# jaymarichua/Applestar

Hardware: AMD Instinct MI355X
Metric: learner samples/sec (AlphaStar policy) (higher is better)
Workload: dtype fp32

## Files before the change

applestar_amd/csrc/bindings.cpp:

```cpp
#include <cstring>
#include <cstdlib>
#include <map>
#include <string>
#include <torch/extension.h>
#include <c10/hip/HIPStream.h>
#include <c10/hip/HIPGuard.h>

#include "kernels.h"

namespace {

hipStream_t stream() { return c10::hip::getCurrentHIPStream().stream(); }

int dt(const at::Tensor& t) {
  if (t.scalar_type() == at::kFloat) return as::DT_F32;
  if (t.scalar_type() == at::kBFloat16) return as::DT_BF16;
  TORCH_CHECK(false, "applestar_amd: unsupported dtype ", t.scalar_type());
}

void check_cuda(const at::Tensor& t, const char* name) {
  TORCH_CHECK(t.is_cuda(), "applestar_amd: ", name, " must be a GPU tensor");
  TORCH_CHECK(t.is_contiguous(), "applestar_amd: ", name, " must be contiguous");
}

// ... 1365 lines not shown
                        static_cast<int>(K), static_cast<int>(act), stream());
  else
    as::gemm_bf16(a.data_ptr(), b.data_ptr(), bp, rp, out.data_ptr(), M, static_cast<int>(N), static_cast<int>(K),
                  static_cast<int>(act), stream());
  return out;
}

at::Tensor gemm_bf16_small(const at::Tensor& a, const at::Tensor& b, const c10::optional<at::Tensor>& bias,
                           const c10::optional<at::Tensor>& res, int64_t act) {
  return gemm_bf16_impl(a, b, bias, res, act, true);
}
at::Tensor gemm_bf16(const at::Tensor& a, const at::Tensor& b, const c10::optional<at::Tensor>& bias,
                     const c10::optional<at::Tensor>& res, int64_t act) {
  return gemm_bf16_impl(a, b, bias, res, act, false);
}

at::Tensor small_gemm(const at::Tensor& a, const at::Tensor& b, const c10::optional<at::Tensor>& bias,
                      const c10::optional<at::Tensor>& res, const c10::optional<at::Tensor>& amask, int64_t mask_mode,
                      int64_t act) {
  check_cuda(a, "a");
  check_cuda(b, "b");
  const bool bf = a.scalar_type() == at::kBFloat16;
  TORCH_CHECK((bf || a.scalar_type() == at::kFloat) && b.scalar_type() == a.scalar_type() && a.dim() == 2 &&
                  b.dim() == 2 && a.is_contiguous() && b.is_contiguous() && a.size(1) == b.size(1),
              "small_gemm: contiguous A [M,K], B [N,K] of one dtype (fp32 / bf16)");
  const int64_t M = a.size(0), K = a.size(1), N = b.size(0);
  TORCH_CHECK(M * K < (1LL << 31) && N * K < (1LL << 31) && M * N < (1LL << 31), "small_gemm: too large");
  TORCH_CHECK(mask_mode >= 0 && mask_mode <= 2 && (act == 0 || act == 1 || act == 2 || act == 4), "small_gemm: codes");
  const float* bp = nullptr;
  if (bias && bias->defined()) {
    TORCH_CHECK(bias->scalar_type() == at::kFloat && bias->numel() == N && bias->is_contiguous() && bias->is_cuda(),
                "small_gemm: fp32 bias [N]");
    bp = bias->data_ptr<float>();
  }
  const void* rp = nullptr;
  if (res && res->defined()) {
    TORCH_CHECK(res->scalar_type() == a.scalar_type() && res->numel() == M * N && res->is_contiguous() && res->is_cuda(),
                "small_gemm: res [M, N] in A's dtype");
    rp = res->data_ptr();
  }
  TORCH_CHECK(act != 4 || rp != nullptr, "small_gemm: the DRELU epilogue masks by res");
  const void* mp = nullptr;
  if (amask && amask->defined() && mask_mode > 0) {
    TORCH_CHECK(amask->scalar_type() == a.scalar_type() && amask->numel() == M * K && amask->is_contiguous() &&
                    amask->is_cuda(), "small_gemm: amask [M, K] in A's dtype");
    mp = amask->data_ptr();
  }
  c10::hip::HIPGuard g(a.device().index());
  auto out = at::empty({M, N}, a.options());
  as::small_nt(a.data_ptr(), b.data_ptr(), bp, rp, mp, static_cast<int>(mask_mode), out.data_ptr(), M,
               static_cast<int>(N), static_cast<int>(K), static_cast<int>(act), bf, stream());
  return out;
}

at::Tensor small_gemm_splitk(const at::Tensor& a, const at::Tensor& b, const c10::optional<at::Tensor>& bias,
                             int64_t act) {
  check_cuda(a, "a");
  check_cuda(b, "b");
  const bool bf = a.scalar_type() == at::kBFloat16;
  TORCH_CHECK((bf || a.scalar_type() == at::kFloat) && b.scalar_type() == a.scalar_type() && a.dim() == 2 &&
                  b.dim() == 2 && a.is_contiguous() && b.is_contiguous() && a.size(1) == b.size(1),
              "small_gemm_splitk: contiguous A [M,K], B [N,K] of one dtype (fp32 / bf16)");
  const int64_t M = a.size(0), K = a.size(1), N = b.size(0);
  TORCH_CHECK(M * K < (1LL << 31) && N * K < (1LL << 31) && M * N < (1LL << 28), "small_gemm_splitk: too large");
  TORCH_CHECK(act == 0 || act == 1 || act == 2, "small_gemm_splitk: act code");
  const float* bp = nullptr;
  if (bias && bias->defined()) {
    TORCH_CHECK(bias->scalar_type() == at::kFloat && bias->numel() == N && bias->is_contiguous() && bias->is_cuda(),
                "small_gemm_splitk: fp32 bias [N]");
    bp = bias->data_ptr<float>();
  }
  c10::hip::HIPGuard g(a.device().index());
  auto out = at::empty({M, N}, a.options());
  const int S = as::small_nt_splits(M, static_cast<int>(N), static_cast<int>(K));
  if (S <= 1) {
    as::small_nt(a.data_ptr(), b.data_ptr(), bp, nullptr, nullptr, 0, out.data_ptr(), M, static_cast<int>(N),
                 static_cast<int>(K), static_cast<int>(act), bf, stream());
    return out;
  }
  auto part = at::empty({S, M, N}, a.options().dtype(at::kFloat));
  as::small_nt_splitk(a.data_ptr(), b.data_ptr(), bp, part.data_ptr<float>(), S, out.data_ptr(), M,
                      static_cast<int>(N), static_cast<int>(K), static_cast<int>(act), bf, stream());
  return out;
}

std::vector<at::Tensor> small_wgrad(const at::Tensor& dy, const at::Tensor& x, const c10::optional<at::Tensor>& ymask,
                                    int64_t mask_mode, bool want_bias, bool out_bf16) {
  check_cuda(dy, "dy");
  check_cuda(x, "x");
  const bool bf = dy.scalar_type() == at::kBFloat16;
  TORCH_CHECK((bf || dy.scalar_type() == at::kFloat) && x.scalar_type() == dy.scalar_type() && dy.dim() == 2 &&
                  x.dim() == 2 && dy.is_contiguous() && x.is_contiguous() && dy.size(0) == x.size(0),
              "small_wgrad: contiguous dy [R, N], x [R, K] of one dtype");
  TORCH_CHECK(!out_bf16 || bf, "small_wgrad: bf16 output needs bf16 inputs");
  TORCH_CHECK(mask_mode >= 0 && mask_mode <= 2, "small_wgrad: mask code");
  const int64_t R = dy.size(0), N = dy.size(1), K = x.size(1);
  TORCH_CHECK(R * N < (1LL << 31) && R * K < (1LL << 31) && N * K < (1LL << 31), "small_wgrad: too large");
  const void* mp = nullptr;
  if (ymask && ymask->defined() && mask_mode > 0) {
    TORCH_CHECK(ymask->scalar_type() == dy.scalar_type() && ymask->numel() == R * N && ymask->is_contiguous() &&
                    ymask->is_cuda(), "small_wgrad: ymask [R, N] in dy's dtype");
    mp = ymask->data_ptr();
  }
  c10::hip::HIPGuard g(dy.device().index());
  auto opts = out_bf16 ? dy.options() : dy.options().dtype(at::kFloat);
  auto dw = at::empty({N, K}, opts);
  at::Tensor db = want_bias ? at::empty({N}, opts) : at::Tensor();
  if (R == 0) {
    dw.zero_();
    if (want_bias) db.zero_();
    return {dw, db};
  }
  as::small_tn(dy.data_ptr(), x.data_ptr(), mp, static_cast<int>(mask_mode), dw.data_ptr(),
               want_bias ? db.data_ptr() : nullptr, R, static_cast<int>(N), static_cast<int>(K), bf, out_bf16, stream());
  return {dw, db};
}

std::vector<at::Tensor> wgrad_f32(const at::Tensor& dy, const at::Tensor& x, int64_t cin, bool want_bias,
                                  const c10::optional<at::Tensor>& out) {
  check_cuda(dy, "dy");
  check_cuda(x, "x");
  TORCH_CHECK(dy.scalar_type() == at::kFloat && x.scalar_type() == at::kFloat, "wgrad_f32: fp32 dy / x");
  TORCH_CHECK(dy.dim() == 2 && dy.is_contiguous() && x.is_contiguous(), "wgrad_f32: contiguous dy [R, N], x");
  const int64_t R = dy.size(0), N = dy.size(1);
  int64_t K, H = 1, W = 1;
  if (cin > 0) {
    TORCH_CHECK(x.dim() == 4 && x.size(3) == cin && x.size(0) * x.size(1) * x.size(2) == R, "wgrad_f32: x NHWC");
    H = x.size(1);
    W = x.size(2);
    K = 9 * cin;
    TORCH_CHECK(cin % 4 == 0, "wgrad_f32: Cin % 4");
  } else {
    TORCH_CHECK(x.dim() == 2 && x.size(0) == R, "wgrad_f32: x [R, K]");
    K = x.size(1);
  }
  TORCH_CHECK(N % 4 == 0 && K % 4 == 0, "wgrad_f32: N and K must be multiples of 4");
  TORCH_CHECK(R * N * 4 < 0x7ffffff0LL && x.numel() * 4 < 0x7ffffff0LL, "wgrad_f32: tensor too large");
  c10::hip::HIPGuard g(dy.device().index());
  auto opts = dy.options();
  const int64_t NK = N * K, stride = NK + (want_bias ? N : 0);
  at::Tensor flat;
  if (out && out->defined()) {
    TORCH_CHECK(out->scalar_type() == at::kFloat && out->is_contiguous() && out->numel() == stride &&
                out->device() == dy.device(), "wgrad_f32: out must be a contiguous fp32 [N K (+ N)] buffer");
    flat = *out;
  }
  if (R == 0) {
    if (flat.defined()) {
      flat.zero_();
      return {flat.narrow(0, 0, NK).view({N, K}), want_bias ? flat.narrow(0, NK, N) : at::Tensor()};
    }
    return {at::zeros({N, K}, opts), want_bias ? at::zeros({N}, opts) : at::Tensor()};
  }
  const int S = as::wgrad_f32_splits(R, static_cast<int>(N), static_cast<int>(K));
  auto part = (S == 1 && flat.defined()) ? flat.view({1, stride}) : at::empty({S, stride}, opts);
  as::wgrad_f32(dy.data_ptr<float>(), x.data_ptr<float>(), part.data_ptr<float>(),
                want_bias ? part.data_ptr<float>() + NK : nullptr, stride, R, static_cast<int>(N), static_cast<int>(K),
                static_cast<int>(H), static_cast<int>(W), static_cast<int>(cin), S, stream());
  if (S == 1) {
    if (!flat.defined()) flat = part.view({stride});
  } else {
    if (!flat.defined()) flat = at::empty({stride}, opts);
    as::column_reduce(part.data_ptr<float>(), flat.data_ptr<float>(), S, static_cast<int>(stride), stream());
  }
  return {flat.narrow(0, 0, NK).view({N, K}), want_bias ? flat.narrow(0, NK, N) : at::Tensor()};
}

std::vector<at::Tensor> wgrad(const at::Tensor& dy, const at::Tensor& x, int64_t cin, bool want_bias, bool bf16_out) {
  check_cuda(dy, "dy");
  check_cuda(x, "x");
  TORCH_CHECK(dy.scalar_type() == at::kBFloat16 && x.scalar_type() == at::kBFloat16, "wgrad: bf16 dy / x");
  TORCH_CHECK(dy.dim() == 2, "wgrad: dy [R, N]");
  TORCH_CHECK(dy.is_contiguous() && x.is_contiguous(), "wgrad: dy and x must be contiguous");
  const int64_t R = dy.size(0), N = dy.size(1);
  int64_t K, H = 1, W = 1;
  if (cin > 0) {
    TORCH_CHECK(x.dim() == 4 && x.size(3) == cin && x.size(0) * x.size(1) * x.size(2) == R, "wgrad: x NHWC");
    H = x.size(1);
    W = x.size(2);
    K = 9 * cin;
    TORCH_CHECK(cin % 8 == 0, "wgrad: Cin % 8");
  } else {
    TORCH_CHECK(x.dim() == 2 && x.size(0) == R, "wgrad: x [R, K]");
    K = x.size(1);
  }
  TORCH_CHECK(N % 8 == 0 && K % 8 == 0, "wgrad: N and K must be multiples of 8");
  TORCH_CHECK(R * N * 2 < 0x7ffffff0LL && x.numel() * 2 < 0x7ffffff0LL, "wgrad: tensor too large");
  c10::hip::HIPGuard g(dy.device().index());
  const int S = R > 0 ? as::wgrad_splits(R, static_cast<int>(N), static_cast<int>(K)) : 1;
  auto opts = dy.options().dtype(at::kFloat);
  if (R == 0) {
    auto zo = bf16_out ? dy.options() : opts;
    return {at::zeros({N, K}, zo), want_bias ? at::zeros({N}, zo) : at::Tensor()};
  }
  const int64_t NK = N * K, stride = NK + (want_bias ? N : 0);
  if (bf16_out && S == 1) {
    auto flat = at::empty({stride}, dy.options());
    as::wgrad(dy.data_ptr(), x.data_ptr(), reinterpret_cast<float*>(flat.data_ptr()),
              want_bias ? reinterpret_cast<float*>(static_cast<at::BFloat16*>(flat.data_ptr()) + NK) : nullptr, 0, R,
              static_cast<int>(N), static_cast<int>(K), static_cast<int>(H), static_cast<int>(W), static_cast<int>(cin),
              1, stream(), true);
    return {flat.narrow(0, 0, NK).view({N, K}), want_bias ? flat.narrow(0, NK, N) : at::Tensor()};
  }
  auto part = at::empty({S, stride}, opts);
  static const bool nan_fill = [] {
    const char* e = std::getenv("APPLESTAR_WGRAD_NANFILL");
    return e != nullptr && e[0] == '1';
  }();
  if (nan_fill) part.fill_(std::numeric_limits<float>::quiet_NaN());
  as::wgrad(dy.data_ptr(), x.data_ptr(), part.data_ptr<float>(), want_bias ? part.data_ptr<float>() + NK : nullptr,
            stride, R, static_cast<int>(N), static_cast<int>(K), static_cast<int>(H), static_cast<int>(W),
            static_cast<int>(cin), S, stream());
  at::Tensor flat;
  if (bf16_out && S <= 1024) {
    flat = at::empty({stride}, dy.options());
    as::column_reduce_bf16(part.data_ptr<float>(), flat.data_ptr(), S, static_cast<int>(stride), stream());
  } else if (S == 1) {
    flat = part.view({stride});
  } else {
    flat = at::empty({stride}, opts);
    as::column_reduce(part.data_ptr<float>(), flat.data_ptr<float>(), S, static_cast<int>(stride), stream());
  }
  if (bf16_out && flat.scalar_type() != at::kBFloat16) flat = flat.to(at::kBFloat16);
  return {flat.narrow(0, 0, NK).view({N, K}), want_bias ? flat.narrow(0, NK, N) : at::Tensor()};
}

namespace {
int idx_code(const at::Tensor& t) {
  if (t.scalar_type() == at::kShort) return 0;
  if (t.scalar_type() == at::kInt) return 1;
  TORCH_CHECK(t.scalar_type() == at::kLong, "bo_encoder: index dtype int16 / int32 / int64");
  return 2;
}

as::BoWeights bo_weights(const std::vector<at::Tensor>& p, int* wdt) {
  TORCH_CHECK(p.size() == 2 + 12 * as::kBoLayers, "bo_encoder: 38 parameter tensors");
  const auto lin_t = p[0].scalar_type();
  TORCH_CHECK(lin_t == at::kFloat || lin_t == at::kBFloat16, "bo_encoder: linear dtype");
  auto lin = [&](const at::Tensor& t, int64_t numel) {
    TORCH_CHECK(t.is_cuda() && t.is_contiguous() && t.scalar_type() == lin_t && t.numel() == numel,
                "bo_encoder: linear parameter (dtype / shape / contiguity)");
    return static_cast<const void*>(t.data_ptr());
  };
  auto ln = [&](const at::Tensor& t) {
    TORCH_CHECK(t.is_cuda() && t.is_contiguous() && t.scalar_type() == at::kFloat && t.numel() == 64,
                "bo_encoder: LayerNorm parameter fp32 [64]");
    return t.data_ptr<float>();
  };
  as::BoWeights w;
  w.w0 = lin(p[0], 64 * 214);
  w.b0 = lin(p[1], 64);
  for (int l = 0; l < as::kBoLayers; ++l) {
    const int o = 2 + 12 * l;
    w.ln1w[l] = ln(p[o]);
    w.ln1b[l] = ln(p[o + 1]);
    w.wqkv[l] = lin(p[o + 2], 48 * 64);
    w.bqkv[l] = lin(p[o + 3], 48);
    w.wp[l] = lin(p[o + 4], 64 * 16);
    w.bp[l] = lin(p[o + 5], 64);
    w.ln2w[l] = ln(p[o + 6]);
    w.ln2b[l] = ln(p[o + 7]);
    w.w1[l] = lin(p[o + 8], 128 * 64);
    w.b1[l] = lin(p[o + 9], 128);
    w.w2[l] = lin(p[o + 10], 64 * 128);
    w.b2[l] = lin(p[o + 11], 64);
  }
  *wdt = lin_t == at::kBFloat16 ? as::DT_BF16 : as::DT_F32;
  return w;
}
}

std::vector<at::Tensor> bo_encoder_fwd(const at::Tensor& bo, const at::Tensor& loc, const std::vector<at::Tensor>& params,
                                       bool save) {
  check_cuda(bo, "bo");
  check_cuda(loc, "loc");
  TORCH_CHECK(bo.dim() == 2 && bo.size(1) == as::kBoTokens && bo.is_contiguous() && loc.sizes() == bo.sizes() &&
                  loc.is_contiguous() && loc.scalar_type() == bo.scalar_type(),
              "bo_encoder: bo / loc [B, 20] contiguous, same dtype");
  int wdt = 0;
  const as::BoWeights w = bo_weights(params, &wdt);
  const int64_t B = bo.size(0);
  c10::hip::HIPGuard g(bo.device().index());
  auto opts = bo.options().dtype(at::kFloat);
  auto out = at::empty({B, 64}, opts);
  at::Tensor rec;
  if (save) rec = at::empty({B, as::kBoLayers, as::kBoRecord}, opts);
  as::bo_encoder_fwd(bo.data_ptr(), loc.data_ptr(), idx_code(bo), w, wdt, out.data_ptr<float>(),
                     save ? rec.data_ptr<float>() : nullptr, B, stream());
  return {out, rec};
}

at::Tensor bo_encoder_bwd(const at::Tensor& bo, const at::Tensor& loc, const std::vector<at::Tensor>& params,
                          const at::Tensor& save, const at::Tensor& dmean, bool ordered) {
  check_cuda(dmean, "dmean");
  const int64_t B = bo.size(0);
  TORCH_CHECK(dmean.scalar_type() == at::kFloat && dmean.is_contiguous() && dmean.numel() == B * 64,
              "bo_encoder_bwd: dmean fp32 [B, 64]");
  TORCH_CHECK(save.scalar_type() == at::kFloat && save.numel() == B * as::kBoLayers * as::kBoRecord,
              "bo_encoder_bwd: saved record");
  int wdt = 0;
  const as::BoWeights w = bo_weights(params, &wdt);
  c10::hip::HIPGuard g(bo.device().index());
  const int reps = static_cast<int>(std::min<int64_t>(B, 32));
  auto rep = at::zeros({reps, as::kBoGradSize}, dmean.options());
  as::bo_encoder_bwd(bo.data_ptr(), loc.data_ptr(), idx_code(bo), w, wdt, save.data_ptr<float>(),
                     dmean.data_ptr<float>(), rep.data_ptr<float>(), B, reps, stream(), ordered);
  auto grad = at::empty({as::kBoGradSize}, dmean.options());
// ... 825 lines not shown
```

applestar_amd/csrc/kernels.h:

```cpp
#pragma once
#include <hip/hip_runtime.h>
#include <stdint.h>

namespace as {

enum DType : int { DT_F32 = 0, DT_BF16 = 1 };
enum SrcType : int { SRC_U8 = 0, SRC_I8 = 1, SRC_I16 = 2, SRC_I32 = 3, SRC_I64 = 4, SRC_F16 = 5, SRC_F32 = 6 };
enum FieldKind : int { FIELD_ONE_HOT = 0, FIELD_BINARY = 1, FIELD_SCALAR = 2 };

constexpr int kMaxFields = 40;
struct EntityFields {
  const void* ptr[kMaxFields];
  int dtype[kMaxFields];
  int kind[kMaxFields];
  int offset[kMaxFields];
  int width[kMaxFields];
  int n;
};

void layer_norm_fwd(const void* x, int x_dt, const void* res, int res_dt, const float* w, const float* b,
                    void* y, int y_dt, float* xsum, float* mean, float* rstd, long rows, int cols, float eps,
                    int act, hipStream_t s);
void layer_norm_bwd(const void* dy, int dy_dt, const void* xin, int xin_dt, const void* y, int y_dt,
                    const float* w, const float* mean, const float* rstd, void* dx, int dx_dt,
// ... 24 lines not shown
void vsp_pool_bwd(const void* dpooled, const uint8_t* pos, const void* pooled, const void* sc, const void* own,
                  const void* enemy, const float* w, void* dsc, float* part, int B, int H, int W, int nblk,
                  hipStream_t s, int dt = DT_BF16);
void vsp_bwd(const void* dout, const void* out, const void* sc, const void* own, const void* enemy, const float* w,
             void* dsc, float* part, long P, int nblk, hipStream_t s, int dt = DT_BF16);
bool loc_in_supported(int C, int P);
void loc_in_fwd(const void* y0, const void* p, const float* wp, void* out, long npix, int HW, hipStream_t s);
int loc_in_bwd_blocks(long npix);
void loc_in_bwd(const void* dy, const void* y, const void* p, const float* wp, void* dym, void* dp, float* part,
                long npix, int HW, int nblk, hipStream_t s);
void gated_residual_bwd(const void* dout, const void* y, const void* g, const float* sp, const void* out,
                        const void* xin, int dt, void* dy, void* dg, void* dx, float* dsp_part, long n, int nblk,
                        hipStream_t s);
int elementwise_blocks(long n);

bool lnlstm_supported(int H);
struct LstmSplit {
  unsigned long long* slab;
  int* err;
};
void lnlstm_fwd(const float* xp, const float* h0, const float* c0, const void* wT, int w_dt, const float* lnh_w,
                const float* lnh_b, const float* lnc_w, const float* lnc_b, int T, int B, int H, float eps, float* out,
                float* c_all, float* xhat_h, float* rstd_h, float* gates, float* xhat_c, float* rstd_c, float* hT,
                float* cT, hipStream_t s, const LstmSplit* split = nullptr, unsigned short* out_bf16 = nullptr);
void lnlstm_bwd(const float* dout, const float* dhT, const float* dcT, const float* gates, const float* c_all,
                const float* xhat_c, const float* rstd_c, const float* xhat_h, const float* rstd_h, const void* w,
                int w_dt, const float* lnh_w, const float* lnc_w, int T, int B, int H, float* dgates, float* dhg,
                float* dc_ln, float* dh0, float* dc0, hipStream_t s, const LstmSplit* split = nullptr);

void entity_embed_fwd(const EntityFields& f, const int64_t* index, const void* wT, int w_dt, const float* bias,
                      void* out, int out_dt, long T, hipStream_t s);
int entity_wgrad_chunks(long T);
void entity_embed_wgrad(const EntityFields& f, const int64_t* index, const void* dout, const void* out, int dt,
                        float* part, long T, int K_in, int nchunk, hipStream_t s);
void entity_onehot(const EntityFields& f, const int64_t* index, void* X, int x_dt, long T, int K_in, hipStream_t s);

struct SpatialPlanes {
  const uint8_t* height;
  const uint8_t* plane[6];
  const int16_t* effect[6];
};
void upsample2x_fwd(const void* x, void* y, int dt, int B, int H, int W, int C, hipStream_t s);
void upsample2x_bwd(const void* dy, void* dx, int dt, int B, int H, int W, int C, hipStream_t s,
                    const void* mask = nullptr);
void spatial_effect_bits(const SpatialPlanes& sp, uint8_t* bits, int B, int L, int HW, hipStream_t s);
void spatial_dense(const SpatialPlanes& sp, const uint8_t* bits, const float* wd, const float* bias, float* pre, long npix,
                   hipStream_t s);
void spatial_dense_input(const SpatialPlanes& sp, const uint8_t* bits, void* X, int x_dt, long npix, hipStream_t s);
void scatter_add_rows(const void* rows, int dt, const uint8_t* ex, const uint8_t* ey, const int64_t* entity_num,
                      float* pre, int B, int N, int H, int W, hipStream_t s);
void gather_rows(const void* dpre, const void* gate, int dt, const uint8_t* ex, const uint8_t* ey,
                 const int64_t* entity_num, void* drows, int B, int N, int H, int W, hipStream_t s);
void relu_cast(const float* x, void* y, int dt, long n, hipStream_t s);
void spatial_embed_fused(const SpatialPlanes& sp, const float* wd, const float* bias, const void* rows, int rows_dt,
                         const uint8_t* ex, const uint8_t* ey, const int64_t* entity_num, void* out, int out_dt, int B,
                         int N, int H, int W, int L, hipStream_t s, bool ordered = false);
bool spatial_pool_supported(int H, int W);
void spatial_embed_pool(const SpatialPlanes& sp, const float* wd, const float* bias, const void* rows, const uint8_t* ex,
                        const uint8_t* ey, const int64_t* entity_num, void* pooled, uint8_t* pos, int B, int N, int H,
                        int W, int L, hipStream_t s, bool f32 = false, bool ordered = false);
int spatial_wgrad_blocks(int B);
void spatial_dense_wgrad(const SpatialPlanes& sp, const void* dpre, const void* gate, int dt, float* part, int B, int H,
                         int W, int L, hipStream_t s);
void spatial_dense_wgrad_pooled(const SpatialPlanes& sp, const float* dy, const float* y, const uint8_t* pos,
                                float* part, int B, int H, int W, int L, hipStream_t s);
void gather_rows_pooled(const float* dy, const float* y, const uint8_t* pos, const uint8_t* ex, const uint8_t* ey,
                        const int64_t* entity_num, float* drows, int B, int N, int H, int W, hipStream_t s);

void varlen_attn_fwd(const void* qkv, const int* cu, void* out, float* lse2, int S, int max_len, int H, long Ttot,
                     float scale, hipStream_t s);
void varlen_attn_bwd(const void* qkv, const void* out, const void* dout, const float* lse2, const int* cu, void* dqkv,
                     float* delta, int S, int max_len, int H, long Ttot, float scale, hipStream_t s);
void varlen_attn_fwd_f32(const float* qkv, const int* cu, float* out, float* lse2, int S, int max_len, int H, long Ttot,
                         float scale, hipStream_t s);
int attn_f32_variant(int v);
void varlen_attn_bwd_f32(const float* qkv, const float* out, const float* dout, const float* lse2, const int* cu,
                         float* dqkv, float* delta, int S, int max_len, int H, long Ttot, float scale, hipStream_t s);

}

namespace as {
void su_sample(const void* key, int key_dt, long key_bstride, const float* c0, const float* u, const int64_t* entity_num,
               const uint8_t* su_mask, const uint16_t* wf, const float* bf, const float* wq2, const float* bq2,
               const float* wih, const float* whh, const float* lni_w, const float* lni_b, const float* lnh_w,
               const float* lnh_b, const float* lnc_w, const float* lnc_b, const float* we1, const float* be1,
               float inv_temp, float eps, int B, int n1_stride, int max_steps, int extra_units, float* logits,
               int64_t* results, float* logp, int64_t* su_num, float* emb, float* extra, hipStream_t s);
}

namespace as {
void segment_copy(const uint8_t* arena, uint8_t* out, const int64_t* seg, long nseg, hipStream_t s);
void conv_wt(const uint16_t* w, uint16_t* out, int cout, int cin, long s0, long s1, long s2, long s3,
             hipStream_t s);
}

namespace as {
int upconv1_channels();
long upconv1_tiles(int B, int Hl, int Wl);
void upconv1_fwd(const void* x, int x_dt, const float* w, const float* bias, float* y, int B, int Hl, int Wl,
                 hipStream_t s);
void upconv1_bwd(const void* x, int x_dt, const float* w, const float* dy, void* dx, float* part, float* dwb, int B,
                 int Hl, int Wl, hipStream_t s, bool relu_mask = false);
}

namespace as {
void maxpool2_fwd(const void* x, void* y, uint8_t* pos, int dt, int B, int H, int W, int C, hipStream_t s);
void maxpool2_bwd(const void* dy, const uint8_t* pos, void* dx, int dt, int B, int H, int W, int C, hipStream_t s,
                  const void* mask = nullptr);
void maxpool2_bwd_relu(const void* dy, const uint8_t* pos, const void* y, void* dx, int B, int H, int W, int C,
                       hipStream_t s, bool f32 = false);
void segment_sum(const void* x, int dt, const int* cu, float* out, int S, int C, hipStream_t s);
void entity_mean_pool(const void* x, int dt, const bool* valid, const void* num, bool num64, void* out, int B, int N,
                      int C, hipStream_t s);
int ln_affine_slices(long R);
void ln_affine_grads(const float* dy, const float* xh, float* part, long R, int C, hipStream_t s);
void table_grad(const void* src, int dt, const int64_t* idx, float* out, long U, int V, int D, hipStream_t s);

bool conv3x3_supported(int Cin, int Cout);
void conv3x3_fwd(const void* x, const void* w, const float* bias, const void* res, void* out, int B, int H, int W,
                 int Cin, int Cout, int act, hipStream_t s);

bool conv3x3_f32_supported(int Cin, int Cout);
void conv3x3_f32_fwd(const float* x, const float* w, const float* bias, const float* res, float* out, int B, int H,
                     int W, int Cin, int Cout, int act, hipStream_t s);
bool conv3x3_f32_epi2_supported(int Cin, int Cout);
void conv3x3_f32_fwd_epi2(const float* x, const float* w, const float* res, const float* res2, long res2_rows,
                          const float* mask, float* out, int B, int H, int W, int Cin, int Cout, hipStream_t s);
int wgrad_f32_splits(long R, int N, int K);
void set_f32_pipe_variant(int v);
int f32_conv_variant();
void set_f32_conv_variant(int v);
int f32_mfma_mode();
void set_f32_mfma_mode(int mode);
void small_nt(const void* a, const void* b, const float* bias, const void* res, const void* amask, int mask_mode,
              void* out, long M, int N, int K, int act, bool bf16, hipStream_t s);
int small_nt_splits(long M, int N, int K);
void small_nt_splitk(const void* a, const void* b, const float* bias, float* part, int S, void* out, long M, int N,
                     int K, int act, bool bf16, hipStream_t s);
void small_tn(const void* dy, const void* x, const void* ymask, int mask_mode, void* dw, void* db, long R, int N,
              int K, bool bf16_in, bool bf16_out, hipStream_t s);
void gemm_bf16_small(const void* a, const void* b, const float* bias, const void* res, void* out, long M, int N, int K,
                     int act, hipStream_t s);
bool gemm_f32_is_small(long M, int N);
void gemm_bf16(const void* a, const void* b, const float* bias, const void* res, void* out, long M, int N, int K,
               int act, hipStream_t s);
void gemm_f32(const float* a, const float* b, const float* bias, const float* res, float* out, long M, int N, int K,
              int act, hipStream_t s);
void wgrad_f32(const float* dy, const float* x, float* dw_part, float* db_part, long part_stride, long R, int N, int K,
               int H, int W, int Cin, int S, hipStream_t st);
int conv_wgrad_halo_f32_mode();
void set_conv_wgrad_halo_f32_mode(int mode);
bool conv_wgrad_f32_halo_supported(int N, int H, int W, int Cin);
bool conv_wgrad_f32_halo_selected(int N, int H, int W, int Cin);
void conv_wgrad_f32_halo(const float* dy, const float* x, float* dw_part, float* db_part, long part_stride, long R,
                         int N, int K, int H, int W, int Cin, int S, long rows_per_split, hipStream_t st);

void head_sample(const void* logits, int logits_dt, long ld_logits, int B, int C, float inv_t, const uint8_t* mask,
                 long mask_ld, const int64_t* lens, const float* u, const void* table, int table_dt,
                 const float* tbias, int D, float* out_logits, int64_t* action, float* emb, hipStream_t s);
void target_unit_sample(const void* e, int e_dt, const float* w1, const float* b1, const float* w2, const float* b2,
                        const void* key, int key_dt, int B, int N, const int64_t* lens, float inv_t, const float* u,
                        float* out_logits, int64_t* action, hipStream_t s);

int fused_adam_chunk();
void fused_clip_adam(const void* table, const long* chunks, int nchunks, int ntensors, float* part,
                     const float* gate, float* norm_out, float max_norm, float* mom, float* scale, float* mom_init,
                     const float* hp, float lr_bc1, float b1, float b2, float inv_sqrt_bc2, float eps, float wd,
                     int decoupled, hipStream_t s);

int wgrad_splits(long R, int N, int K);

constexpr int kCopyMaxT = 64;
constexpr long kCopyChunk = 8192;
constexpr long kCopyRawChunk = 16384;
struct CopyArgs {
  int ntensors;
  int chunk_start[kCopyMaxT + 1];
  const void* src[kCopyMaxT];
  void* dst[kCopyMaxT];
  long n[kCopyMaxT];
  unsigned char dts[kCopyMaxT];
};
void multi_copy(const CopyArgs& a, hipStream_t s);

constexpr int kColMaxP = 32;
struct ColSumArgs {
  int npieces;
  long rows;
  int block_start[kColMaxP + 1];
  float* dst[kColMaxP];
  int dld[kColMaxP], doff[kColMaxP], width[kColMaxP], nsrc[kColMaxP];
  const float* src[kColMaxP][3];
  int sld[kColMaxP][3], soff[kColMaxP][3];
};
void col_sum(const ColSumArgs& a, hipStream_t s);

constexpr int kLogpMaxH = 8;
struct LogpArgs {
  int nheads;
  long row_start[kLogpMaxH + 1];
  const void* logits[kLogpMaxH];
  const int64_t* action[kLogpMaxH];
  float* out[kLogpMaxH];
  int cols[kLogpMaxH];
  unsigned char bf16[kLogpMaxH];
  long blk_start[kLogpMaxH + 1];
  unsigned char big[kLogpMaxH];
};
void multi_logp(const LogpArgs& a, hipStream_t s);

long presplit_b_bytes(int N, int K);
void presplit_b(const float* b, int N, int K, bool trans, void* out, hipStream_t s);
bool gemm_f32_psb_supported(long M, int N, int K);
constexpr int kPresplitMax = 48;
struct PresplitArgs {
  int n;
  int block_start[kPresplitMax + 1];
  const float* src[kPresplitMax];
  void* dst[kPresplitMax];
  int N[kPresplitMax], K[kPresplitMax];
  unsigned char trans[kPresplitMax];
};
void multi_presplit(const PresplitArgs& a, hipStream_t s);
void gemm_f32_psb(const float* a, const void* bsplit, const float* bias, const float* res, float* out, long M, int N,
                  int K, int act, int variant, hipStream_t s);
bool conv3x3_f32_psb_supported(long M, int Cin, int Cout);
void conv3x3_f32_psb(const float* x, const void* wsplit, const float* bias, const float* res, const float* res2,
                     long res2_rows, const float* mask, float* out, int B, int H, int W, int Cin, int Cout, int act,
                     hipStream_t s);
void conv3x3_f32_psb_stream(const float* x, const void* wsplit, const float* bias, const float* res,
                            const float* res2, long res2_rows, const float* mask, float* out, int B, int H, int W,
                            int Cin, int Cout, int act, hipStream_t s);
void conv3x3_f32_v2(const float* x, const void* wsplit, const float* bias, const float* res, const float* res2,
                    long res2_rows, const float* mask, float* out, int B, int H, int W, int Cin, int Cout, int act,
                    int variant, hipStream_t s);
void gemm_f32_v2(const float* a, const void* bsplit, const float* bias, const float* res, float* out, long M, int N,
                 int K, int act, int variant, hipStream_t s);
bool conv3x3_f32_halo_supported(int H, int W, int Cin, int Cout);
bool conv3x3_f32_halo_selected(int H, int W, int Cin, int Cout);
int conv_halo_f32_mode();
void set_conv_halo_f32_mode(int mode);
void conv3x3_f32_halo(const float* x, const void* wsplit, const float* bias, const float* res, const float* res2,
                      long res2_rows, const float* mask, float* out, int B, int H, int W, int Cin, int Cout, int act,
                      hipStream_t s);

constexpr int kSCopyMaxT = 24;
struct StridedCopyArgs {
  int ntensors;
  int chunk_start[kSCopyMaxT + 1];
  const void* src[kSCopyMaxT];
  void* dst[kSCopyMaxT];
  int n[kSCopyMaxT];
  int size[kSCopyMaxT][4];
  long stride[kSCopyMaxT][4];
  long base[kSCopyMaxT];
  unsigned char dts[kSCopyMaxT];
};
void multi_strided_copy(const StridedCopyArgs& a, hipStream_t s);

bool pointwise_supported(int cin, int cout);
void pointwise_conv(const void* x, const float* w, const float* bias, void* y, long P, int cin, int cout, int act,
                    hipStream_t s);

void act_grad_nhwc(const void* dout, int dt, bool dout_nchw, const void* out, void* dpre, int B, int C, int HW, int relu,
                   hipStream_t s);
void wgrad(const void* dy, const void* x, float* dw_part, float* db_part, long part_stride, long R, int N, int K,
           int H, int W, int Cin, int S, hipStream_t st, bool out_bf16 = false);
constexpr int kWgMaxBatch = 32;
struct WgBatch {
  const void* dy[kWgMaxBatch];
  const void* x[kWgMaxBatch];
  float* dw[kWgMaxBatch];
  float* db[kWgMaxBatch];
};
void wgrad_batched(const WgBatch& P, int nb, long part_stride, long R, int N, int K, int H, int W, int Cin, int S,
                   hipStream_t st, bool out_bf16 = false);

constexpr int kBoTokens = 20, kBoLayers = 3, kBoRecord = 11120, kBoGradSize = 76880;
struct BoWeights {
  const void* w0;
  const void* b0;
  const float* ln1w[kBoLayers];
  const float* ln1b[kBoLayers];
  const void* wqkv[kBoLayers];
  const void* bqkv[kBoLayers];
  const void* wp[kBoLayers];
  const void* bp[kBoLayers];
  const float* ln2w[kBoLayers];
  const float* ln2b[kBoLayers];
  const void* w1[kBoLayers];
  const void* b1[kBoLayers];
  const void* w2[kBoLayers];
  const void* b2[kBoLayers];
};
void bo_encoder_fwd(const void* bo, const void* loc, int idt, const BoWeights& w, int wdt, float* out, float* save,
                    long B, hipStream_t st);
void bo_encoder_bwd(const void* bo, const void* loc, int idt, const BoWeights& w, int wdt, const float* save,
                    const float* dmean, float* grad, long B, int replicas, hipStream_t st, bool ordered = false);

void mm_k32(const void* a, const void* wT, void* out, long R, int N, hipStream_t s);

constexpr int kResMax = 16;
struct ResMlpW {
  const void* w1[kResMax];
  const void* b1[kResMax];
  const void* w2[kResMax];
// ... 72 lines not shown
```

applestar_amd/csrc/kernels/conv_wgrad_f32_halo.hip:

```cpp
#include <cstdlib>

#include "../common.h"
#include "../kernels.h"
#include "../split_mfma.h"
#include "../f32_pipe.h"
#include "../conv_tap.h"

namespace as {
namespace {

using pipe::f16v;

constexpr int kWgBN = 128, kWgCC = 32, kWgRS = 16, kWgMaxW = 80;

typedef short s16x4 __attribute__((ext_vector_type(4)));
typedef __attribute__((address_space(3))) s16x4 lds_s16x4;

template <int WMAX>
struct WgHaloCfg {
  static constexpr int SA = kWgBN * 2 + 64, SX = kWgCC * 2;
  static constexpr int NRING = 2 * kWgRS + 2 * WMAX + 2 <= 128 ? 128 : 256;
  static constexpr int PA = kWgRS * SA;
  static constexpr int PX = (NRING + 1) * SX;
  static constexpr int SMEM = 6 * PA + 3 * PX;
// ... 62 lines not shown
  const int x_base = static_cast<int>(((r_begin + W + 1 + x_row) * Cin + c0 + 4 * x_q) * 4);
  const long x_left = R - (r_begin + W + 1 + x_row);
  const int x_lim = (x_colok && x_wave && x_left > 0) ? static_cast<int>(x_left) : 0;
  const int x_step = RS * Cin * 4;
  const bool do_bias = db_part != nullptr && ch == 0;
  const int b_col = n0 + (tid & 127), b_h = tid >> 7;
  const int b_base = static_cast<int>(((r_begin + 8 * b_h) * N + b_col) * 4);
  const int b_lim = b_col < N ? nrows - 8 * b_h : 0;
  float rb[8], bsum = 0.f;
  uint4 ra[2], rx;
  auto load_stage = [&](int j) {
    if (do_bias) {
#pragma unroll
      for (int q = 0; q < 8; ++q)
        rb[q] = __uint_as_float(__builtin_amdgcn_raw_buffer_load_b32(
            yr, j * RS + q < b_lim ? b_base + j * a_step + q * N * 4 : kOOB, 0, 0));
    }
#pragma unroll
    for (int i = 0; i < 2; ++i) {
      const auto v =
          __builtin_amdgcn_raw_buffer_load_b128(yr, j * RS < a_lim[i] ? a_base[i] + j * a_step : kOOB, 0, 0);
      ra[i] = make_uint4(v[0], v[1], v[2], v[3]);
    }
    const auto v = __builtin_amdgcn_raw_buffer_load_b128(xr, j * RS < x_lim ? x_base + j * x_step : kOOB, 0, 0);
    rx = make_uint4(v[0], v[1], v[2], v[3]);
  };
  auto add_bias = [&]() {
    if (do_bias) {
#pragma unroll
      for (int q = 0; q < 8; ++q) bsum += rb[q];
    }
  };
  const int a_dst = a_row * SA + a_q * 8;
  const int x_dst0 = (2 * (W + 1) + x_row) * SX + x_q * 8;
  auto store_stage = [&](int j) {
#pragma unroll
    for (int i = 0; i < 2; ++i) split_store(pa + (j & 1) * 3 * C::PA, C::PA, a_dst + 8 * i * SA, ra[i]);
    add_bias();
    if (x_wave) split_store(px, C::PX, (x_dst0 + j * RS * SX) & (RINGB - 1), rx);
  };

  const int g = lane >> 4, tq = (lane >> 2) & 3, tp = lane & 3;
  const int rr0 = 8 * (g >> 1) + tq;
  const int a_off = rr0 * SA + (32 * wid + 16 * (g & 1) + 4 * tp) * 2;
  const int x_col = (16 * (g & 1) + 4 * tp) * 2;
  const int x_off0 = (W + 1 + rr0) * SX + x_col;
  const int x_zero = RINGB + x_col;
  int shb[9];
#pragma unroll
  for (int t = 0; t < 9; ++t) shb[t] = ((t / 3 - 1) * W + (t % 3 - 1)) * SX;
  int py[2], pxx[2];
#pragma unroll
  for (int r = 0; r < 2; ++r) {
    const int rem = static_cast<int>((r_begin + rr0 + 4 * r) % HW);
    py[r] = rem / W;
    pxx[r] = rem - py[r] * W;
  }
  const int adv = RS % HW, adv_y = adv / W, adv_x = adv - adv_y * W;

  f16v acc[9];
#pragma unroll
  for (int t = 0; t < 9; ++t)
#pragma unroll
    for (int e = 0; e < 16; ++e) acc[t][e] = 0.f;

  for (int i = tid; i < 3 * SX / 4; i += 256)
    *reinterpret_cast<unsigned*>(px + (i / (SX / 4)) * C::PX + RINGB + (i % (SX / 4)) * 4) = 0u;
  load_stage(0);
  {
    const int npieces = (RS + 2 * W + 2) * (CC / 4);
    for (int piece = tid; piece < npieces; piece += 256) {
      const int row = piece >> 3;
      const long pix = r_begin - (W + 1) + row;
      const bool ok = x_colok && pix >= 0 && pix < R;
      const auto v = __builtin_amdgcn_raw_buffer_load_b128(
          xr, ok ? (static_cast<int>(pix) * Cin + c0 + 4 * x_q) * 4 : kOOB, 0, 0);
      split_store(px, C::PX, row * SX + x_q * 8, make_uint4(v[0], v[1], v[2], v[3]));
    }
  }
  {
#pragma unroll
    for (int i = 0; i < 2; ++i) split_store(pa, C::PA, a_dst + 8 * i * SA, ra[i]);
    add_bias();
  }
  __syncthreads();

  for (int j = 0; j < nsteps; ++j) {
    const bool more = j + 1 < nsteps;
    if (more) load_stage(j + 1);
    int ok[2];
#pragma unroll
    for (int r = 0; r < 2; ++r) {
      ok[r] = conv_tap_mask_yx(py[r], pxx[r], H, W);
      pxx[r] += adv_x;
      py[r] += adv_y;
      if (pxx[r] >= W) { pxx[r] -= W; ++py[r]; }
      if (py[r] >= H) py[r] -= H;
    }
    const char* ap = pa + (j & 1) * 3 * C::PA + a_off;
    Split3 fa;
#pragma unroll
    for (int p = 0; p < 3; ++p) fa.p[p] = tr_frag(ap + p * C::PA, ap + p * C::PA + 4 * SA);
    const int xs = x_off0 + j * RS * SX;
    auto read_x = [&](int t) {
      const int m0 = __builtin_amdgcn_sbfe(ok[0], t, 1), m1 = __builtin_amdgcn_sbfe(ok[1], t, 1);
      const int o0 = (((xs + shb[t]) & (RINGB - 1)) & m0) | (x_zero & ~m0);
      const int o1 = (((xs + 4 * SX + shb[t]) & (RINGB - 1)) & m1) | (x_zero & ~m1);
      Split3 f;
#pragma unroll
      for (int p = 0; p < 3; ++p) f.p[p] = tr_frag(px + p * C::PX + o0, px + p * C::PX + o1);
      return f;
    };
    Split3 fb[2];
    fb[0] = read_x(0);
#pragma unroll
    for (int t = 0; t < 9; ++t) {
      if (t + 1 < 9) fb[(t + 1) & 1] = read_x(t + 1);
      __builtin_amdgcn_sched_barrier(0);
      acc[t] = mfma_x6(fa, fb[t & 1], acc[t]);
      __builtin_amdgcn_sched_barrier(0);
    }
    if (more) store_stage(j + 1);
    __syncthreads();
  }

  float* outp = dw_part + static_cast<long>(s) * part_stride;
  const int c = c0 + l32;
  if (c < Cin) {
#pragma unroll
    for (int t = 0; t < 9; ++t)
#pragma unroll
      for (int e = 0; e < 16; ++e) {
        const int n = n0 + 32 * wid + (e & 3) + 8 * (e >> 2) + 4 * h;
        if (n < N) outp[static_cast<long>(n) * K + t * Cin + c] = acc[t][e];
      }
  }
  if (do_bias) {
    float* red = reinterpret_cast<float*>(smem);
    red[tid] = bsum;
    __syncthreads();
    if (b_h == 0 && b_col < N) db_part[static_cast<long>(s) * part_stride + b_col] = bsum + red[tid + 128];
  }
}

template <int WMAX>
void launch_wg_halo(const float* dy, const float* x, float* dwp, float* dbp, long ps, long R, int N, int K, int H,
                    int W, int Cin, int S, long rps, hipStream_t st) {
  const int tiles_n = (N + kWgBN - 1) / kWgBN, chunks = (Cin + kWgCC - 1) / kWgCC;
  const long nwg = static_cast<long>(S) * tiles_n * chunks;
  hipLaunchKernelGGL((conv_wgrad_f32_halo_kernel<WMAX>), dim3(static_cast<unsigned>(nwg)), dim3(256), 0, st, dy, x,
                     dwp, dbp, ps, R, N, K, H, W, Cin, rps, tiles_n, chunks);
}

int& wg_halo_ref() {
  static int v = [] {
    const char* e = std::getenv("APPLESTAR_CONV_WGRAD_HALO_F32");
    return e ? std::atoi(e) & 7 : 4;
  }();
  return v;
}

}

int conv_wgrad_halo_f32_mode() { return wg_halo_ref(); }
void set_conv_wgrad_halo_f32_mode(int mode) { wg_halo_ref() = mode & 7; }

bool conv_wgrad_f32_halo_supported(int N, int H, int W, int Cin) {
  return f32_mfma_mode() == 1 && H > 0 && W > 0 && W <= kWgMaxW && Cin > 0 && Cin % 16 == 0 && N > 0 && N % 128 == 0;
}

bool conv_wgrad_f32_halo_selected(int N, int H, int W, int Cin) {
  const int bit = N == 32 ? 1 : (N == 64 ? 2 : 4);
  return (conv_wgrad_halo_f32_mode() & bit) != 0 && conv_wgrad_f32_halo_supported(N, H, W, Cin);
}

void conv_wgrad_f32_halo(const float* dy, const float* x, float* dw_part, float* db_part, long part_stride, long R,
                         int N, int K, int H, int W, int Cin, int S, long rows_per_split, hipStream_t st) {
  if (W <= 40) launch_wg_halo<40>(dy, x, dw_part, db_part, part_stride, R, N, K, H, W, Cin, S, rows_per_split, st);
  else launch_wg_halo<kWgMaxW>(dy, x, dw_part, db_part, part_stride, R, N, K, H, W, Cin, S, rows_per_split, st);
}

}
```

Measured before the change: 8525.

## Add narrow-N halo conv weight-gradient kernel and enable it for N<=64

Adds a specialised fp32 conv weight-gradient kernel for narrow output-channel counts (N up to 32 or 64). Each workgroup covers the full N and splits the rows and warps differently, with a 3-stage split-precision LDS ring for the input halo. A new split heuristic targets a fixed workgroup count, and the default mode now enables the halo path for all N classes, replacing the generic im2col-style wgrad for these small convolutions. It adds a cross-wave reduction through LDS and more partial buffers, which a column reduce then combines.

```diff
diff --git a/applestar_amd/csrc/bindings.cpp b/applestar_amd/csrc/bindings.cpp
--- a/applestar_amd/csrc/bindings.cpp
+++ b/applestar_amd/csrc/bindings.cpp
@@ -1541,7 +1541,9 @@
     }
     return {at::zeros({N, K}, opts), want_bias ? at::zeros({N}, opts) : at::Tensor()};
   }
-  const int S = as::wgrad_f32_splits(R, static_cast<int>(N), static_cast<int>(K));
+  const int S = cin > 0 ? as::conv_wgrad_f32_splits(R, static_cast<int>(N), static_cast<int>(K), static_cast<int>(H),
+                                                    static_cast<int>(W), static_cast<int>(cin))
+                        : as::wgrad_f32_splits(R, static_cast<int>(N), static_cast<int>(K));
   auto part = (S == 1 && flat.defined()) ? flat.view({1, stride}) : at::empty({S, stride}, opts);
   as::wgrad_f32(dy.data_ptr<float>(), x.data_ptr<float>(), part.data_ptr<float>(),
                 want_bias ? part.data_ptr<float>() + NK : nullptr, stride, R, static_cast<int>(N), static_cast<int>(K),
diff --git a/applestar_amd/csrc/kernels.h b/applestar_amd/csrc/kernels.h
--- a/applestar_amd/csrc/kernels.h
+++ b/applestar_amd/csrc/kernels.h
@@ -200,6 +200,7 @@
 void set_conv_wgrad_halo_f32_mode(int mode);
 bool conv_wgrad_f32_halo_supported(int N, int H, int W, int Cin);
 bool conv_wgrad_f32_halo_selected(int N, int H, int W, int Cin);
+int conv_wgrad_f32_splits(long R, int N, int K, int H, int W, int Cin);
 void conv_wgrad_f32_halo(const float* dy, const float* x, float* dw_part, float* db_part, long part_stride, long R,
                          int N, int K, int H, int W, int Cin, int S, long rows_per_split, hipStream_t st);
 
diff --git a/applestar_amd/csrc/kernels/conv_wgrad_f32_halo.hip b/applestar_amd/csrc/kernels/conv_wgrad_f32_halo.hip
--- a/applestar_amd/csrc/kernels/conv_wgrad_f32_halo.hip
+++ b/applestar_amd/csrc/kernels/conv_wgrad_f32_halo.hip
@@ -238,31 +238,290 @@
                      dwp, dbp, ps, R, N, K, H, W, Cin, rps, tiles_n, chunks);
 }
 
+template <int WN>
+struct WgNarrowCfg {
+  static constexpr int WR = 4 / WN, RS = 16 * WR, BN = 32 * WN;
+  static constexpr int SA = BN == 32 ? 64 : BN * 2 + 64, SX = kWgCC * 2;
+  static constexpr int NRING = 256;
+  static constexpr int PA = RS * SA, PX = (NRING + 1) * SX;
+  static constexpr int SMEM = 3 * PA + 3 * PX;
+  static constexpr int TH = 5;
+  static_assert(RS + 2 * kWgMaxW + 2 <= NRING && 2 * SMEM <= 160 * 1024, "ring size / two workgroups per CU");
+  static_assert(WN * TH * 16 * 64 * 4 <= SMEM && 256 * 4 * 4 <= SMEM, "the final sums reuse the planes");
+};
+
+template <int WN>
+__global__ __launch_bounds__(256, 2) void conv_wgrad_f32_halo_narrow_kernel(
+    const float* __restrict__ dy, const float* __restrict__ x, float* __restrict__ dw_part,
+    float* __restrict__ db_part, long part_stride, long R, int N, int K, int H, int W, int Cin, long rows_per_split,
+    int chunks) {
+  using C = WgNarrowCfg<WN>;
+  constexpr int RS = C::RS, BN = C::BN, CC = kWgCC, SA = C::SA, SX = C::SX, WR = C::WR;
+  constexpr int RINGB = C::NRING * SX;
+  constexpr int AQ = BN / 4, AROWS = 256 / AQ;
+  constexpr int XP = RS / 32;
+  static_assert(2 * AROWS == RS, "two dY pieces per thread");
+  __shared__ __attribute__((aligned(16))) char smem[C::SMEM];
+  char* const pa = smem;
+  char* const px = smem + 3 * C::PA;
+
+  const int wg = pipe::xcd_remap();
+  const int ch = wg % chunks;
+  const int s = wg / chunks;
+  const int c0 = ch * CC;
+  const long r_begin = static_cast<long>(s) * rows_per_split;
+  const long r_end = r_begin + rows_per_split < R ? r_begin + rows_per_split : R;
+  const int tid = threadIdx.x, lane = tid & 63, wid = __builtin_amdgcn_readfirstlane(tid >> 6);
+  const int wn = wid % WN, wr = wid / WN;
+  const int l32 = lane & 31, h = lane >> 5;
+  const int HW = H * W;
+  const __amdgpu_buffer_rsrc_t yr =
+      __builtin_amdgcn_make_buffer_rsrc(const_cast<float*>(dy), 0, static_cast<int>(R * N * 4), 0x00020000);
+  const __amdgpu_buffer_rsrc_t xr =
+      __builtin_amdgcn_make_buffer_rsrc(const_cast<float*>(x), 0, static_cast<int>(R * Cin * 4), 0x00020000);
+  const int nrows = r_end > r_begin ? static_cast<int>(r_end - r_begin) : 0;
+  const int nsteps = (nrows + RS - 1) / RS;
+
+  const int a_q = tid % AQ, a_row = tid / AQ;
+  const bool a_colok = 4 * a_q < N;
+  int a_base[2], a_lim[2];
+#pragma unroll
+  for (int i = 0; i < 2; ++i) {
+    a_base[i] = static_cast<int>(((r_begin + a_row + AROWS * i) * N + 4 * a_q) * 4);
+    a_lim[i] = a_colok ? nrows - (a_row + AROWS * i) : 0;
+  }
+  const int a_step = RS * N * 4;
+  const int x_q = tid & 7, x_row = tid >> 3;
+  const bool x_colok = c0 + 4 * x_q < Cin;
+  int x_base[XP], x_lim[XP];
+#pragma unroll
+  for (int i = 0; i < XP; ++i) {
+    const long pix = r_begin + W + 1 + x_row + 32 * i;
+    x_base[i] = static_cast<int>((pix * Cin + c0 + 4 * x_q) * 4);
+    x_lim[i] = (x_colok && R - pix > 0) ? static_cast<int>(R - pix) : 0;
+  }
+  const int x_step = RS * Cin * 4;
+  const bool do_bias = db_part != nullptr && ch == 0;
+  float bs[4] = {0.f, 0.f, 0.f, 0.f};
+  uint4 ra[2], rx[XP];
+  auto load_stage = [&](int j) {
+#pragma unroll
+    for (int i = 0; i < 2; ++i) {
+      const auto v =
+          __builtin_amdgcn_raw_buffer_load_b128(yr, j * RS < a_lim[i] ? a_base[i] + j * a_step : kOOB, 0, 0);
+      ra[i] = make_uint4(v[0], v[1], v[2], v[3]);
+    }
+#pragma unroll
+    for (int i = 0; i < XP; ++i) {
+      const auto v =
+          __builtin_amdgcn_raw_buffer_load_b128(xr, j * RS < x_lim[i] ? x_base[i] + j * x_step : kOOB, 0, 0);
+      rx[i] = make_uint4(v[0], v[1], v[2], v[3]);
+    }
+  };
+  const int a_dst = a_row * SA + a_q * 8;
+  auto store_a = [&]() {
+#pragma unroll
+    for (int i = 0; i < 2; ++i) {
+      split_store(pa, C::PA, a_dst + AROWS * i * SA, ra[i]);
+      bs[0] += __uint_as_float(ra[i].x);
+      bs[1] += __uint_as_float(ra[i].y);
+      bs[2] += __uint_as_float(ra[i].z);
+      bs[3] += __uint_as_float(ra[i].w);
+    }
+  };
+  const int x_dst0 = (2 * (W + 1) + x_row) * SX + x_q * 8;
+  auto store_stage = [&](int j) {
+    store_a();
+#pragma unroll
+    for (int i = 0; i < XP; ++i) split_store(px, C::PX, (x_dst0 + (j * RS + 32 * i) * SX) & (RINGB - 1), rx[i]);
+  };
+
+  const int g = lane >> 4, tq = (lane >> 2) & 3, tp = lane & 3;
+  const int rr0 = 16 * wr + 8 * (g >> 1) + tq;
+  const int a_off = rr0 * SA + (32 * wn + 16 * (g & 1) + 4 * tp) * 2;
+  const int x_col = (16 * (g & 1) + 4 * tp) * 2;
+  const int x_off0 = (W + 1 + rr0) * SX + x_col;
+  const int x_zero = RINGB + x_col;
+  int shb[9];
+#pragma unroll
+  for (int t = 0; t < 9; ++t) shb[t] = ((t / 3 - 1) * W + (t % 3 - 1)) * SX;
+  int py[2], pxx[2];
+#pragma unroll
+  for (int r = 0; r < 2; ++r) {
+    const int rem = static_cast<int>((r_begin + rr0 + 4 * r) % HW);
+    py[r] = rem / W;
+    pxx[r] = rem - py[r] * W;
+  }
+  const int adv = RS % HW, adv_y = adv / W, adv_x = adv - adv_y * W;
+
+  f16v acc[9];
+#pragma unroll
+  for (int t = 0; t < 9; ++t)
+#pragma unroll
+    for (int e = 0; e < 16; ++e) acc[t][e] = 0.f;
+
+  for (int i = tid; i < 3 * SX / 4; i += 256)
+    *reinterpret_cast<unsigned*>(px + (i / (SX / 4)) * C::PX + RINGB + (i % (SX / 4)) * 4) = 0u;
+  load_stage(0);
+  {
+    const int npieces = (RS + 2 * W + 2) * (CC / 4);
+    for (int piece = tid; piece < npieces; piece += 256) {
+      const int row = piece >> 3;
+      const long pix = r_begin - (W + 1) + row;
+      const bool ok = x_colok && pix >= 0 && pix < R;
+      const auto v = __builtin_amdgcn_raw_buffer_load_b128(
+          xr, ok ? (static_cast<int>(pix) * Cin + c0 + 4 * x_q) * 4 : kOOB, 0, 0);
+      split_store(px, C::PX, row * SX + x_q * 8, make_uint4(v[0], v[1], v[2], v[3]));
+    }
+  }
+  store_a();
+  __syncthreads();
+
+  for (int j = 0; j < nsteps; ++j) {
+    const bool more = j + 1 < nsteps;
+    if (more) load_stage(j + 1);
+    int ok[2];
+#pragma unroll
+    for (int r = 0; r < 2; ++r) {
+      ok[r] = conv_tap_mask_yx(py[r], pxx[r], H, W);
+      pxx[r] += adv_x;
+      py[r] += adv_y;
+      if (pxx[r] >= W) { pxx[r] -= W; ++py[r]; }
+      if (py[r] >= H) py[r] -= H;
+    }
+    const char* ap = pa + a_off;
+    Split3 fa;
+#pragma unroll
+    for (int p = 0; p < 3; ++p) fa.p[p] = tr_frag(ap + p * C::PA, ap + p * C::PA + 4 * SA);
+    const int xs = x_off0 + j * RS * SX;
+    auto read_x = [&](int t) {
+      const int m0 = __builtin_amdgcn_sbfe(ok[0], t, 1), m1 = __builtin_amdgcn_sbfe(ok[1], t, 1);
+      const int o0 = (((xs + shb[t]) & (RINGB - 1)) & m0) | (x_zero & ~m0);
+      const int o1 = (((xs + 4 * SX + shb[t]) & (RINGB - 1)) & m1) | (x_zero & ~m1);
+      Split3 f;
+#pragma unroll
+      for (int p = 0; p < 3; ++p) f.p[p] = tr_frag(px + p * C::PX + o0, px + p * C::PX + o1);
+      return f;
+    };
+    Split3 fb[2];
+    fb[0] = read_x(0);
+#pragma unroll
+    for (int t = 0; t < 9; ++t) {
+      if (t + 1 < 9) fb[(t + 1) & 1] = read_x(t + 1);
+      __builtin_amdgcn_sched_barrier(0);
+      acc[t] = mfma_x6(fa, fb[t & 1], acc[t]);
+      __builtin_amdgcn_sched_barrier(0);
+    }
+    if (more) {
+      __syncthreads();
+      store_stage(j + 1);
+    }
+    __syncthreads();
+  }
+
+  float* const red = reinterpret_cast<float*>(smem);
+#pragma unroll
+  for (int r = 1; r < WR; ++r)
+#pragma unroll
+    for (int t0 = 0; t0 < 9; t0 += C::TH) {
+      if (wr == r) {
+#pragma unroll
+        for (int t = t0; t < t0 + C::TH && t < 9; ++t)
+#pragma unroll
+          for (int e = 0; e < 16; ++e) red[((wn * C::TH + t - t0) * 16 + e) * 64 + lane] = acc[t][e];
+      }
+      __syncthreads();
+      if (wr == 0) {
+#pragma unroll
+        for (int t = t0; t < t0 + C::TH && t < 9; ++t)
+#pragma unroll
+          for (int e = 0; e < 16; ++e) acc[t][e] += red[((wn * C::TH + t - t0) * 16 + e) * 64 + lane];
+      }
+      __syncthreads();
+    }
+
+  float* outp = dw_part + static_cast<long>(s) * part_stride;
+  const int c = c0 + l32;
+  if (wr == 0 && c < Cin) {
+#pragma unroll
+    for (int t = 0; t < 9; ++t)
+#pragma unroll
+      for (int e = 0; e < 16; ++e) {
+        const int n = 32 * wn + (e & 3) + 8 * (e >> 2) + 4 * h;
+        if (n < N) outp[static_cast<long>(n) * K + t * Cin + c] = acc[t][e];
+      }
+  }
+  if (do_bias) {
+#pragma unroll
+    for (int q = 0; q < 4; ++q) red[a_row * BN + 4 * a_q + q] = bs[q];
+    __syncthreads();
+    if (tid < N) {
+      float v = red[tid];
+      for (int i = 1; i < AROWS; ++i) v += red[i * BN + tid];
+      db_part[static_cast<long>(s) * part_stride + tid] = v;
+    }
+  }
+}
+
+template <int WN>
+void launch_wg_halo_narrow(const float* dy, const float* x, float* dwp, float* dbp, long ps, long R, int N, int K,
+                           int H, int W, int Cin, int S, long rps, hipStream_t st) {
+  const int chunks = (Cin + kWgCC - 1) / kWgCC;
+  const long nwg = static_cast<long>(S) * chunks;
+  hipLaunchKernelGGL((conv_wgrad_f32_halo_narrow_kernel<WN>), dim3(static_cast<unsigned>(nwg)), dim3(256), 0, st, dy,
+                     x, dwp, dbp, ps, R, N, K, H, W, Cin, rps, chunks);
+}
+
 int& wg_halo_ref() {
   static int v = [] {
     const char* e = std::getenv("APPLESTAR_CONV_WGRAD_HALO_F32");
-    return e ? std::atoi(e) & 7 : 4;
+    return e ? std::atoi(e) & 7 : 7;
   }();
   return v;
 }
 
+long wg_halo_narrow_target() {
+  static const long v = [] {
+    const char* e = std::getenv("APPLESTAR_CONV_WGRAD_HALO_WG");
+    const long x = e ? std::atol(e) : 512;
+    return x >= 1 ? x : 512;
+  }();
+  return v;
+}
+
 }
 
 int conv_wgrad_halo_f32_mode() { return wg_halo_ref(); }
 void set_conv_wgrad_halo_f32_mode(int mode) { wg_halo_ref() = mode & 7; }
 
 bool conv_wgrad_f32_halo_supported(int N, int H, int W, int Cin) {
-  return f32_mfma_mode() == 1 && H > 0 && W > 0 && W <= kWgMaxW && Cin > 0 && Cin % 16 == 0 && N > 0 && N % 128 == 0;
+  return f32_mfma_mode() == 1 && H > 0 && W > 0 && W <= kWgMaxW && Cin > 0 && Cin % 16 == 0 && N > 0 &&
+         (N % 128 == 0 || (N <= 64 && N % 4 == 0));
 }
 
 bool conv_wgrad_f32_halo_selected(int N, int H, int W, int Cin) {
-  const int bit = N == 32 ? 1 : (N == 64 ? 2 : 4);
+  const int bit = N <= 32 ? 1 : (N <= 64 ? 2 : 4);
   return (conv_wgrad_halo_f32_mode() & bit) != 0 && conv_wgrad_f32_halo_supported(N, H, W, Cin);
+}
+
+int conv_wgrad_f32_splits(long R, int N, int K, int H, int W, int Cin) {
+  if (!(N <= 64 && conv_wgrad_f32_halo_selected(N, H, W, Cin))) return wgrad_f32_splits(R, N, K);
+  const long chunks = (Cin + kWgCC - 1) / kWgCC, rs = N <= 32 ? WgNarrowCfg<1>::RS : WgNarrowCfg<2>::RS;
+  long S = (wg_halo_narrow_target() + chunks - 1) / chunks;
+  const long max_s = (R + 2 * rs - 1) / (2 * rs);
+  if (S > max_s) S = max_s;
+  const long max_part = (16L << 20) / (static_cast<long>(N) * K);
+  if (S > max_part) S = max_part;
+  if (S < 1) S = 1;
+  return static_cast<int>(S);
 }
 
 void conv_wgrad_f32_halo(const float* dy, const float* x, float* dw_part, float* db_part, long part_stride, long R,
                          int N, int K, int H, int W, int Cin, int S, long rows_per_split, hipStream_t st) {
-  if (W <= 40) launch_wg_halo<40>(dy, x, dw_part, db_part, part_stride, R, N, K, H, W, Cin, S, rows_per_split, st);
+  if (N <= 32) launch_wg_halo_narrow<1>(dy, x, dw_part, db_part, part_stride, R, N, K, H, W, Cin, S, rows_per_split, st);
+  else if (N <= 64)
+    launch_wg_halo_narrow<2>(dy, x, dw_part, db_part, part_stride, R, N, K, H, W, Cin, S, rows_per_split, st);
+  else if (W <= 40) launch_wg_halo<40>(dy, x, dw_part, db_part, part_stride, R, N, K, H, W, Cin, S, rows_per_split, st);
   else launch_wg_halo<kWgMaxW>(dy, x, dw_part, db_part, part_stride, R, N, K, H, W, Cin, S, rows_per_split, st);
 }
 
```

After: 8723, median of 6. 2.3% higher.
